# mhnazeri/PMoE

Hardware: AMD Instinct MI355X
Metric: samples/sec fwd+bwd, 256x256 RGB 4-expert PMoE (higher is better)
Workload: dtype bf16; 1 GPU; 4-expert MoE (PMoE experts), 256x256x3 x4 frames, batch 64/GPU, fwd+moe_loss+bwd, dropout 0.3; global_batch=64, parallelism=dp1

## Files before the change

pmoe_amd/csrc/api.hip:

```cpp
#include "common.h"
#include "kernels.h"

static ConvArgs to_args(const pmoe_conv_desc* d) {
    ConvArgs a;
    a.in = d->in; a.w = d->w; a.out = d->out; a.res = d->res; a.bias = d->bias; a.stats = d->stats;
    a.N = d->n; a.H = d->h; a.W = d->w_; a.Cin = d->cin;
    a.Ho = d->ho; a.Wo = d->wo; a.Cout = d->cout; a.CoutP = d->coutp;
    a.in_ld = d->in_ld; a.in_coff = d->in_coff; a.out_ld = d->out_ld; a.out_coff = d->out_coff;
    a.res_ld = d->res_ld; a.res_coff = d->res_coff;
    a.ipe = d->ipe; a.in_shared = d->in_shared;
    a.ks = d->ks; a.stride = d->stride; a.pad = d->pad; a.dilate = d->dilate;
    a.act = d->act; a.res_mode = (d->res || d->res_mode == PMOE_RES_INBN) ? d->res_mode : PMOE_RES_NONE;
    a.drop_p = d->drop_p; a.seed = d->seed;
    a.oscale = d->out_scale; a.in_scale = d->in_scale; a.w_fp8 = d->w_fp8; a.in_fp8 = d->in_fp8;
    a.bn = d->bn_coef; a.bn_ipe = d->bn_ipe > 0 ? d->bn_ipe : d->ipe;
    a.lTW = a.lTH = a.TN = a.n_groups = a.tiles_y = a.tiles_x = 0;
    a.kh = a.kw = d->ks; a.use_tapmap = 0; a.tapmap[0] = a.tapmap[1] = a.tapmap[2] = a.tapmap[3] = 0;
    a.out_step = 1; a.out_offy = a.out_offx = 0; a.OH = d->ho; a.OW = d->wo; a.prefetch = 0; a.stagger = 0;
    a.shuf_c = d->shuffle_c > 0 ? d->shuffle_c : 0;
    return a;
}

static int check_conv(const pmoe_conv_desc* d) {
    if (!d || !d->in || !d->w || !d->out) return PMOE_ERR_ARG;
    if (d->n <= 0 || d->h <= 0 || d->w_ <= 0 || d->ho <= 0 || d->wo <= 0 || d->ipe <= 0) return PMOE_ERR_ARG;
    const int ve = d->dtype == PMOE_DT_BF16 ? 8 : 4;
    if (d->in_fp8 && (!d->w_fp8 || d->dtype != PMOE_DT_BF16 || d->in_ld % 16 || d->in_coff % 16)) return PMOE_ERR_ARG;
    if (d->in_ld % ve || d->in_coff % ve || d->out_ld % ve || d->out_coff % ve) return PMOE_ERR_ARG;
    if (d->res && (d->res_ld % ve || d->res_coff % ve)) return PMOE_ERR_ARG;
    if (d->shuffle_c > 0 ? (d->cout != 4 * d->shuffle_c || d->shuffle_c % ve || d->out_coff + d->shuffle_c > d->out_ld || d->cout > d->coutp)
                         : (d->cout > d->coutp || d->out_coff + d->cout > d->out_ld)) return PMOE_ERR_ARG;
    if (d->in_coff + d->cin > d->in_ld) return PMOE_ERR_ARG;
    if (d->drop_p < 0.f || d->drop_p >= 1.f) return PMOE_ERR_ARG;
    if (d->res && d->res_mode == PMOE_RES_DBN &&
        (!d->bn_coef || !d->stats || d->dtype != PMOE_DT_BF16 || (d->bn_ipe > 0 && (d->bn_ipe % d->ipe || d->n % d->bn_ipe))))
        return PMOE_ERR_ARG;
    if (d->res_mode == PMOE_RES_INBN &&
        (d->res || !d->bn_coef || d->dtype != PMOE_DT_BF16 || (d->bias && d->ks != 1) || d->act != PMOE_ACT_NONE || d->drop_p != 0.f || d->in_shared ||
         d->w_fp8 || d->dilate || (d->bn_ipe > 0 && (d->bn_ipe % d->ipe || d->n % d->bn_ipe))))
        return PMOE_ERR_ARG;
    if (!d->dilate) {
        if (d->ho != (d->h + 2 * d->pad - d->ks) / d->stride + 1) return PMOE_ERR_ARG;
        if (d->wo != (d->w_ + 2 * d->pad - d->ks) / d->stride + 1) return PMOE_ERR_ARG;
    }
    return 0;
}

extern "C" {

int pmoe_version(void) { return PMOE_ABI_VERSION; }

int pmoe_abi_sizeof(int which) {
    return which == 0 ? (int)sizeof(pmoe_conv_desc) : which == 1 ? (int)sizeof(pmoe_wgrad_desc)
           : which == 2 ? (int)sizeof(pmoe_opt_tensor) : which == 3 ? (int)sizeof(pmoe_opt_pack)
           : which == 4 ? (int)sizeof(pmoe_aug_plan) : PMOE_ERR_ARG;
}

const char* pmoe_error_string(int code) {
    if (code == 0) return "ok";
    if (code == PMOE_ERR_ARG) return "pmoe: invalid argument (shape / alignment / pointer)";
    if (code == PMOE_ERR_UNSUPPORTED) return "pmoe: unsupported configuration (no tile fits LDS)";
    if (code > 0) return hipGetErrorString((hipError_t)code);
    return "pmoe: unknown error";
}

int pmoe_conv2d_igemm(const pmoe_conv_desc* d, void* stream) {
    int rc = check_conv(d);
    if (rc) return rc;
    return conv_igemm_launch(to_args(d), d->dtype, (hipStream_t)stream);
}

static ConvArgs to_plan_args(const pmoe_conv_desc* d) {
    ConvArgs a = to_args(d);
    if (a.in_ld <= 0) a.in_ld = a.in_coff + a.Cin;
    if (a.out_ld <= 0) a.out_ld = a.out_coff + a.Cout;
    return a;
}

int pmoe_conv2d_stat_rows(const pmoe_conv_desc* d) {
    if (!d || d->ipe <= 0) return PMOE_ERR_ARG;
    return conv_igemm_mblocks(to_plan_args(d), d->dtype);
}

int pmoe_conv2d_plan(const pmoe_conv_desc* d) {
    if (!d || d->ipe <= 0) return PMOE_ERR_ARG;
    return conv_igemm_plan(to_plan_args(d), d->dtype);
}

static int to_wgrad_args(const pmoe_wgrad_desc* d, WgradArgs& a) {
    if (!d || d->ipe <= 0) return PMOE_ERR_ARG;
    const int ve = d->dtype == PMOE_DT_BF16 ? 8 : 4;
    if (d->x_ld % ve || d->x_coff % ve || d->dy_ld % ve || d->dy_coff % ve) return PMOE_ERR_ARG;
    if (d->x_coff + d->cin > d->x_ld || d->dy_coff + d->cout > d->dy_ld) return PMOE_ERR_ARG;
// ... 47 lines not shown
```

pmoe_amd/csrc/conv_c16.hip:

```cpp
#include "common.h"
#include "kernels.h"

namespace {

typedef unsigned v4u __attribute__((ext_vector_type(4)));
typedef float f32x2 __attribute__((ext_vector_type(2)));

__global__ void __launch_bounds__(256, 2) conv3x3_c16_kernel(ConvArgs a, int tiles_x, int tiles_per_expert, int wgs_per_expert,
                                                            unsigned in_bytes, unsigned out_bytes) {
    __shared__ v4i wl[18][64];
    __shared__ v4i tbuf[4][256];
    __shared__ float red[4][8][2][64];
    const int tid = threadIdx.x, lane = tid & 63;
    const int wave = __builtin_amdgcn_readfirstlane(tid >> 6);
    const int e = blockIdx.y, wg = blockIdx.x;
    {
        const bf16* w = reinterpret_cast<const bf16*>(a.w) + (size_t)e * a.CoutP * 9 * 16;
        for (int idx = tid; idx < 18 * 64; idx += 256) {
            const int l = idx & 63, mtap = idx >> 6, mt = mtap / 9, tap = mtap - mt * 9;
            const int m = l & 31, kh = l >> 5;
            const int aa = m >> 3, hh = (m >> 2) & 1, b = m & 3;
            const int cout = 16 * (2 * mt + (aa >> 1)) + 8 * hh + 4 * (aa & 1) + b;
            wl[mtap][l] = ldg16(w + ((size_t)cout * 9 + tap) * 16 + kh * 8);
        }
    }
    __syncthreads();
    const size_t in_img0 = a.in_shared ? 0 : (size_t)e * a.ipe, out_img0 = (size_t)e * a.ipe;
    const __amdgpu_buffer_rsrc_t rs_in = __builtin_amdgcn_make_buffer_rsrc(
        (void*)(reinterpret_cast<const bf16*>(a.in) + in_img0 * a.H * a.W * a.in_ld + a.in_coff - a.in_ld), (short)0,
        (int)(in_bytes + (unsigned)a.in_ld * 2u), 0x00020000);
    const __amdgpu_buffer_rsrc_t rs_out = __builtin_amdgcn_make_buffer_rsrc(
        (void*)(reinterpret_cast<bf16*>(a.out) + out_img0 * a.H * a.W * a.out_ld + a.out_coff), (short)0, (int)out_bytes, 0x00020000);
    constexpr unsigned OOB = 0xfffffff0u;
    const int px_l = lane & 31, kh = lane >> 5;
    const unsigned ld2 = (unsigned)a.in_ld * 2u, old2 = (unsigned)a.out_ld * 2u;
    const unsigned vin = (unsigned)(px_l + 1) * ld2 + (unsigned)kh * 16u;
    unsigned vout[4];
#pragma unroll
    for (int i = 0; i < 4; ++i) vout[i] = (unsigned)(i * 8 + (lane >> 3)) * old2 + (unsigned)(lane & 7) * 16u;
    const bool chunk_ok = (lane & 7) * 8 < a.Cout;
    const int t0 = (int)((long long)tiles_per_expert * wg / wgs_per_expert);
    const int t1 = (int)((long long)tiles_per_expert * (wg + 1) / wgs_per_expert);
    f32x2 s1[4], s2[4];
#pragma unroll
    for (int j = 0; j < 4; ++j) s1[j] = s2[j] = f32x2{0.f, 0.f};

    struct Pos { int xt, y, img; };
    auto advance = [&](Pos& p) {
        p.xt += 4;
        while (p.xt >= tiles_x) { p.xt -= tiles_x; if (++p.y == a.H) { p.y = 0; ++p.img; } }
    };
    auto load_tile = [&](const Pos& p, v4u (&raw)[9], bool live) {
        const unsigned row0 = ((unsigned)(p.img * a.H + p.y) * (unsigned)a.W + (unsigned)p.xt * 32u) * ld2;
        const int px = p.xt * 32 + px_l;
        unsigned vq[3];
        vq[0] = live && px >= 1 && px - 1 < a.W ? vin - ld2 : OOB;
        vq[1] = live && px < a.W ? vin : OOB;
        vq[2] = live && px + 1 < a.W ? vin + ld2 : OOB;
#pragma unroll
        for (int r = 0; r < 3; ++r) {
            const int yy = p.y + r - 1;
            const bool row_ok = live && (unsigned)yy < (unsigned)a.H;
            const unsigned soff = row_ok ? row0 + (unsigned)(r - 1) * (unsigned)a.W * ld2 : 0u;
#pragma unroll
            for (int q = 0; q < 3; ++q)
                raw[r * 3 + q] = __builtin_amdgcn_raw_buffer_load_b128(rs_in, (int)(row_ok ? vq[q] : OOB), (int)soff, 0);
        }
    };
    auto process = [&](const Pos& pc, const v4u (&cur)[9]) {
        f32x16 acc[2];
#pragma unroll
        for (int mt = 0; mt < 2; ++mt)
#pragma unroll
            for (int i = 0; i < 16; ++i) acc[mt][i] = 0.f;
#pragma unroll
        for (int tap = 0; tap < 9; ++tap)
#pragma unroll
            for (int mt = 0; mt < 2; ++mt)
                acc[mt] = __builtin_amdgcn_mfma_f32_32x32x16_bf16(__builtin_bit_cast(bf16x8, wl[mt * 9 + tap][lane]),
                                                                  __builtin_bit_cast(bf16x8, cur[tap]), acc[mt], 0, 0, 0);
#pragma unroll
        for (int g = 0; g < 4; ++g) {
            float v[8];
#pragma unroll
            for (int i = 0; i < 8; ++i) v[i] = acc[g >> 1][8 * (g & 1) + i];
            tbuf[wave][px_l * 8 + ((2 * g + kh) ^ (px_l & 7))] = pack16<bf16>(v);
        }
        const unsigned osoff = ((unsigned)(pc.img * a.H + pc.y) * (unsigned)a.W + (unsigned)pc.xt * 32u) * old2;
#pragma unroll
        for (int i = 0; i < 4; ++i) {
            const int p = i * 8 + (lane >> 3), c = lane & 7;
            const v4i v = tbuf[wave][p * 8 + (c ^ (p & 7))];
            const bool ok = pc.xt * 32 + p < a.W;
            __builtin_amdgcn_raw_buffer_store_b128(__builtin_bit_cast(v4u, v), rs_out, (int)(ok && chunk_ok ? vout[i] : OOB), (int)osoff, 0);
            if (a.stats && ok) {
                float rr[8];
                unpack16<bf16>(v, rr);
#pragma unroll
                for (int q = 0; q < 4; ++q) {
                    const f32x2 r2 = f32x2{rr[2 * q], rr[2 * q + 1]};
                    s1[q] += r2;
                    s2[q] = __builtin_elementwise_fma(r2, r2, s2[q]);
                }
            }
        }
    };
    Pos pl, pc;
    {
        const int t = t0 + wave;
        pl.xt = t % tiles_x;
        const int r = t / tiles_x;
        pl.y = r % a.H;
        pl.img = r / a.H;
        pc = pl;
    }
    v4u b0[9], b1[9], b2[9];
    int tl = t0 + wave, t = tl;
    auto fetch = [&](v4u (&buf)[9]) {
        load_tile(pl, buf, tl < t1);
        advance(pl);
        tl += 4;
    };
    fetch(b0);
    fetch(b1);
    while (t < t1) {
        fetch(b2);
        process(pc, b0); advance(pc); t += 4;
        if (t >= t1) break;
        fetch(b0);
        process(pc, b1); advance(pc); t += 4;
        if (t >= t1) break;
        fetch(b1);
        process(pc, b2); advance(pc); t += 4;
    }
    if (!a.stats) return;
#pragma unroll
    for (int q = 0; q < 8; ++q) {
        red[wave][lane >> 3][0][(lane & 7) * 8 + q] = s1[q >> 1][q & 1];
        red[wave][lane >> 3][1][(lane & 7) * 8 + q] = s2[q >> 1][q & 1];
    }
    __syncthreads();
    if (tid < 128) {
        const int which = tid >> 6, c = tid & 63;
        float s = 0.f;
        for (int w = 0; w < 4; ++w)
            for (int pg = 0; pg < 8; ++pg) s += red[w][pg][which][c];
        a.stats[(((size_t)e * wgs_per_expert + wg) * 2 + which) * a.CoutP + c] = s;
    }
}

}

bool conv_c16_plan(const ConvArgs& a, int dtype, ConvLaunch* l) {
    if (!sw("PMOE_CONV_C16", 1)) return false;
    if (dtype != PMOE_DT_BF16 || a.w_fp8 || a.ks != 3 || a.stride != 1 || a.pad != 1 || a.dilate) return false;
    if (a.Cin != 16 || a.CoutP != 64 || a.Cout % 8 || a.Cout > 64) return false;
    if (a.bias || a.act != PMOE_ACT_NONE || a.res_mode != PMOE_RES_NONE || a.drop_p > 0.f) return false;
    if (a.N % a.ipe || a.Ho != a.H || a.Wo != a.W) return false;
    if (a.in_ld % 8 || a.in_coff % 8 || a.out_ld % 8 || a.out_coff % 8) return false;
    if ((long long)a.ipe * a.H * a.W * (a.in_ld > a.out_ld ? a.in_ld : a.out_ld) * 2 >= 0xfff00000ll) return false;
    const int E = a.N / a.ipe, tx = (a.W + 31) / 32;
    const long long tpe = (long long)a.ipe * a.H * tx;
    if (tpe > 0x7fffffffll || tpe < 64) return false;
    int wpe = 512 / E;
    if (wpe < 1) wpe = 1;
    if (wpe > tpe / 16) wpe = (int)(tpe / 16);
    if (wpe < 1) wpe = 1;
    l->kind = CONV_C16; l->code = 1316; l->a = a;
    l->wpe = wpe; l->tiles_x = tx; l->tpe = (int)tpe; l->mblocks = E * wpe;
    return true;
}

int conv_c16_launch(const ConvLaunch& l, hipStream_t st) {
    const ConvArgs& a = l.a;
    const long long in_b = (long long)a.ipe * a.H * a.W * a.in_ld * 2 - (long long)a.in_coff * 2;
    const long long out_b = (long long)a.ipe * a.H * a.W * a.out_ld * 2 - (long long)a.out_coff * 2;
    return launch<conv3x3_c16_kernel, 0>(dim3(l.wpe, a.N / a.ipe), dim3(256), 0, st, a, l.tiles_x, l.tpe, l.wpe, (unsigned)in_b, (unsigned)out_b);
}
```

pmoe_amd/csrc/conv_igemm.hip:

```cpp
#include "conv_common.h"
#include <stdlib.h>
#include <string.h>
#include "kernels.h"

template <int LOG_RB> __device__ __forceinline__ int swz(int x) { return swz_chunk<LOG_RB, 0>(x); }

template <typename T> struct Mma;
template <> struct Mma<bf16> {
    static __device__ __forceinline__ void run(const v4i& a, const v4i& b, f32x16& c) {
        c = __builtin_amdgcn_mfma_f32_32x32x16_bf16(__builtin_bit_cast(bf16x8, a), __builtin_bit_cast(bf16x8, b), c, 0, 0, 0);
    }
};
template <> struct Mma<float> {
    static __device__ __forceinline__ void run(const v4i& a, const v4i& b, f32x16& c) {
        const f32x4 fa = __builtin_bit_cast(f32x4, a), fb = __builtin_bit_cast(f32x4, b);
#pragma unroll
        for (int j = 0; j < 4; ++j) c = __builtin_amdgcn_mfma_f32_32x32x2f32(fa[j], fb[j], c, 0, 0, 0);
    }
};

template <> struct Mma<fp8> {
    static __device__ __forceinline__ void run(const v4i& a, const v4i& b, f32x16& c) {
        typedef long l2 __attribute__((ext_vector_type(2)));
        const l2 la = __builtin_bit_cast(l2, a), lb = __builtin_bit_cast(l2, b);
// ... 404 lines not shown
        l->smem = smem;
        l->log_rb = log_rb; l->lite = lite;
        l->wm = big || !wide ? 4 : 2; l->wn = wide ? 2 : 1;
        l->code = (F8 ? 8000 : 0) + (lite ? 2000 + log_rb : log_rb * 100 + l->wm * 10 + l->wn);
        return 0;
    }
    return PMOE_ERR_UNSUPPORTED;
}

static int tile_plan_dtype(const ConvArgs& a, int dtype, ConvLaunch* l) {
    return dtype == PMOE_DT_BF16 ? tile_plan(a, 2, 2, l) : dtype == PMOE_DT_F32 ? tile_plan(a, 4, 4, l) : PMOE_ERR_ARG;
}

template <typename T, typename TL = T> static int tile_launch(const ConvLaunch& l, hipStream_t st) {
    const ConvArgs& a = l.a;
    if (l.lite) return launch_lite<T, 7, TL>(a, l.mblocks, l.smem, st);
    switch (l.log_rb * 100 + l.wm * 10 + l.wn) {
    case 742: return launch_cfg<T, 7, 4, 2, TL>(a, l.mblocks, l.smem, st);
    case 642: return launch_cfg<T, 6, 4, 2, TL>(a, l.mblocks, l.smem, st);
    case 722: return launch_cfg<T, 7, 2, 2, TL>(a, l.mblocks, l.smem, st);
    case 741: return launch_cfg<T, 7, 4, 1, TL>(a, l.mblocks, l.smem, st);
    case 622: return launch_cfg<T, 6, 2, 2, TL>(a, l.mblocks, l.smem, st);
    case 641: return launch_cfg<T, 6, 4, 1, TL>(a, l.mblocks, l.smem, st);
    }
    if constexpr (sizeof(TL) == sizeof(T)) {
        switch (l.log_rb * 100 + l.wm * 10 + l.wn) {
        case 542: return launch_cfg<T, 5, 4, 2>(a, l.mblocks, l.smem, st);
        case 522: return launch_cfg<T, 5, 2, 2>(a, l.mblocks, l.smem, st);
        case 541: return launch_cfg<T, 5, 4, 1>(a, l.mblocks, l.smem, st);
        }
    }
    return PMOE_ERR_UNSUPPORTED;
}

static int launch_one(const ConvLaunch& l, int dtype, hipStream_t st) {
    switch (l.kind) {
    case CONV_SKINNY: return gemm_skinny_launch(l, st);
    case CONV_C16: return conv_c16_launch(l, st);
    case CONV_C1X1: return conv_c1x1_launch(l, st);
    case CONV_RES: return conv_res_launch(l, st);
    case CONV_DMA: case CONV_DMA_S2: case CONV_DMA_S2CLS: case CONV_DMA_F8: return conv_dma_launch(l, st);
    case CONV_TILE:
        if (l.a.w_fp8) return !l.a.oscale || !(l.a.in_scale > 0.f) ? PMOE_ERR_ARG : tile_launch<bf16, fp8>(l, st);
        return dtype == PMOE_DT_BF16 ? tile_launch<bf16>(l, st) : tile_launch<float>(l, st);
    }
    return PMOE_ERR_ARG;
}

static int select_stride2_dgrad(const ConvArgs& a, int dtype, ConvPlan* p) {
    p->n = 0;
    for (int py = 0; py < 2; ++py)
        for (int px = 0; px < 2; ++px) {
            ConvArgs c = a;
            c.dilate = 0; c.stride = 1; c.pad = 0;
            c.kh = 1 + py; c.kw = 1 + px;
            c.Ho = (a.Ho - py + 1) / 2; c.Wo = (a.Wo - px + 1) / 2;
            if (c.Ho <= 0 || c.Wo <= 0) continue;
            c.OH = a.Ho; c.OW = a.Wo; c.out_step = 2; c.out_offy = py; c.out_offx = px;
            c.use_tapmap = 1;
            for (int r = 0; r < c.kh; ++r)
                for (int q = 0; q < c.kw; ++q) {
                    const int fy = py ? (r == 0 ? 0 : 2) : 1, fx = px ? (q == 0 ? 0 : 2) : 1;
                    c.tapmap[r * c.kw + q] = fy * 3 + fx;
                }
            ConvLaunch* l = &p->l[p->n++];
            if (!conv_dma_s2cls_plan(c, dtype, l)) {
                const int rc = tile_plan_dtype(c, dtype, l);
                if (rc) return rc;
            }
        }
    if (!p->n) return PMOE_ERR_ARG;
    ConvLaunch t;
    const int esz = dtype == PMOE_DT_BF16 ? 2 : 4, rc = tile_plan(a, esz, esz, &t);
    p->mblocks = rc ? rc : t.mblocks;
    return 4000 + p->l[p->n - 1].code;
}

int conv_select(const ConvArgs& a, int dtype, ConvPlan* p) {
    memset(p, 0, sizeof(*p));
    p->n = 1;
    ConvLaunch* l = p->l;
    int code = 0;
    const bool bn_mode = a.res_mode == PMOE_RES_INBN || a.res_mode == PMOE_RES_DBN;
    if (a.in_fp8 && !a.w_fp8) {
        code = PMOE_ERR_UNSUPPORTED;
    } else if (a.shuf_c) {
        code = conv_c1x1_plan(a, dtype, l) ? 0 : PMOE_ERR_UNSUPPORTED;
    } else if (a.w_fp8) {
        if (dtype != PMOE_DT_BF16 || a.dilate) code = PMOE_ERR_ARG;
        else if (a.in_fp8) code = conv_dma_f8_plan(a, dtype, l) ? 0 : PMOE_ERR_UNSUPPORTED;
        else if (bn_mode) code = PMOE_ERR_UNSUPPORTED;
        else code = tile_plan(a, 2, 1, l);
    } else if (a.res_mode == PMOE_RES_INBN) {
        if (!(!a.bias && conv_res_plan(a, dtype, l) && l->res_pipe) && !conv_c1x1_plan(a, dtype, l))
            code = PMOE_ERR_UNSUPPORTED;
    } else if (a.res_mode == PMOE_RES_DBN) {
        if (!(conv_res_plan(a, dtype, l) && l->res_dma) && (gemm_skinny_plan(a, dtype, l) || !conv_dma_plan(a, dtype, l)))
            code = PMOE_ERR_UNSUPPORTED;
    } else if (a.dilate && a.ks == 3 && a.pad == 1 && a.kh == 3) {
        const int code = select_stride2_dgrad(a, dtype, p);
        if (code < 0) p->n = 0;
        return p->code = code;
    } else if (a.dilate && a.ks == 1 && a.pad == 0 && a.res_mode == PMOE_RES_ADD && a.res == a.out && a.res_ld == a.out_ld &&
               a.res_coff == a.out_coff && !a.bias && a.act == PMOE_ACT_NONE && a.drop_p == 0.f) {
        ConvArgs c = a;
        c.dilate = 0; c.stride = 1; c.pad = 0; c.kh = c.kw = 1;
        c.Ho = (a.Ho + 1) / 2; c.Wo = (a.Wo + 1) / 2;
        c.OH = a.Ho; c.OW = a.Wo; c.out_step = 2; c.out_offy = c.out_offx = 0;
        code = tile_plan_dtype(c, dtype, l);
    } else if (!gemm_skinny_plan(a, dtype, l) && !conv_c16_plan(a, dtype, l) && !conv_c1x1_plan(a, dtype, l) &&
               !conv_res_plan(a, dtype, l) && !conv_dma_plan(a, dtype, l) && !conv_dma_s2_plan(a, dtype, l)) {
        code = tile_plan_dtype(a, dtype, l);
    }
    if (code < 0) { p->n = 0; return p->code = code; }
    p->mblocks = l->mblocks;
    return p->code = l->code;
}

int conv_igemm_launch(const ConvArgs& a, int dtype, hipStream_t st) {
    ConvPlan p;
    const int code = conv_select(a, dtype, &p);
    if (code < 0) return code;
    for (int i = 0; i < p.n; ++i) {
        const int rc = launch_one(p.l[i], dtype, st);
        if (rc) return rc;
    }
    return 0;
}

int conv_igemm_plan(const ConvArgs& a, int dtype) {
    ConvPlan p;
    return conv_select(a, dtype, &p);
}

int conv_igemm_mblocks(const ConvArgs& a, int dtype) {
    static float rows_only;
    ConvArgs s = a;
    if (!s.stats) s.stats = &rows_only;
    ConvPlan p;
    const int code = conv_select(s, dtype, &p);
    return code < 0 ? code : p.mblocks;
}
```

pmoe_amd/engine.py:

```python
import collections
import itertools
import os

import torch
import torch.distributed as dist

from . import hip, ops
from .model import blocks as B
from .parallel import BucketedAllReduce

F32 = torch.float32


def r16(c):
    return (c + 15) // 16 * 16


def r64(c):
    return (c + 63) // 64 * 64


class BNCoef:
    __slots__ = ("block", "mean", "invstd", "scale", "shift", "rpe")

    def __init__(self, E, C_, rpe, dev):
        self.block, self.rpe = torch.empty(4, E, C_, dtype=F32, device=dev), rpe
        self.mean, self.invstd, self.scale, self.shift = self.block.unbind(0)


class Partials(collections.namedtuple("Partials", "t rows E")):
    __slots__ = ()

    @classmethod
    def of_epilogue(cls, stats, E):
        return cls(stats, stats.shape[0] // E, E)

    def fold(self, width, cap=128):
        if self.rows <= cap:
            return self
        small = torch.empty(self.E, 128, width, dtype=F32, device=self.t.device)
        ops.reduce_partials(self.t, small, self.E, self.rows, 128, width)
        return Partials(small, 128, self.E)


BNSource = collections.namedtuple("BNSource", "z layer coef")
BNFused = collections.namedtuple("BNFused", "g coef c1 c2")


class Var:
    __slots__ = ("t", "coff", "c", "g", "needs_grad", "act", "drop_p", "base", "gap_part", "bn_src", "bn_part", "f8", "bn_defer",
                 "bn_fused", "pending_bn", "sink")

    def __init__(self, t, c=None, coff=0, needs_grad=False, base=None):
        self.t, self.coff, self.c = t, coff, (c if c is not None else t.shape[-1])
        self.g, self.needs_grad, self.act, self.drop_p, self.base = None, needs_grad, hip.ACT_NONE, 0.0, base
        self.gap_part = None
        self.bn_src = None
        self.bn_part = None
        self.f8 = None
        self.bn_defer = False
        self.bn_fused = None
        self.pending_bn = None
        self.sink = None

    @property
    def grad(self):
        return self.base.g if self.base is not None else self.g

    def set_grad(self, g):
        if (self.base if self.base is not None else self).bn_part is not None:
            raise RuntimeError("relu(BatchNorm(z)) whose backward reductions came out of its consumer's data gradient "
                               "(PMOE_RES_DBN) takes exactly one consumer; a second gradient contribution arrived")
        if self.base is not None:
            self.base.g = g
        else:
            self.g = g

    def window(self, coff, c):
        return Var(self.t, c, coff, self.needs_grad, base=self if self.base is None else self.base)


PackSinks = collections.namedtuple("PackSinks", "gen by_param")


class GroupedConv:
    scatter_grads = None
    route_bias = True

    def __init__(self, eng, name, weights, biases, cin, cout, ks, stride, pad):
        self.eng, self.name = eng, name
        self.weights, self.biases = weights, biases
        self.cin, self.cout, self.ks, self.stride, self.pad = cin, cout, ks, stride, pad
        self.cinp, self.coutp, self.cout_st = r16(cin), r64(cout), r16(cout)
        self.dg_rows, self.dg_red = r64(cin), r16(cout)
# ... 874 lines not shown
        self._arena_numel = (off + 255) // 256 * 256

    def _bucket_cuts(self, n_buckets):
        tail = None
        for key in self._order:
            layer = next((l for k, l, _ in self.params if self._key(k, l) == key), None)
            name = getattr(layer, "name", "")
            if name.startswith("layer1.") or name.startswith("stem.") or name in ("bn1", "eca1", "eca2"):
                tail = self._slots[key][0]
                break
        n = self._arena_numel
        if tail is None or tail <= 0 or n_buckets < 2:
            b = (n + n_buckets - 1) // n_buckets
            return [min(n, (i + 1) * ((b + 255) // 256 * 256)) for i in range(n_buckets)]
        tail = tail // 256 * 256
        b = (tail + n_buckets - 2) // (n_buckets - 1)
        b = (b + 255) // 256 * 256
        return [min(tail, (i + 1) * b) for i in range(n_buckets - 1)] + [n]

    def _grad_slot(self, kind, layer):
        key = self._key(kind, layer)
        off, n, _ = self._slots[key]
        self._filled.add(key)
        return self._arena[off:off + n]

    def _final_prefix(self):
        while self._cursor < len(self._order):
            key = self._order[self._cursor]
            _, _, plist = self._slots[key]
            if key in self._filled or not any(p.requires_grad for p in plist):
                self._cursor += 1
            else:
                break
        if self._cursor == len(self._order):
            return self._arena_numel
        return self._slots[self._order[self._cursor]][0]

    def _begin(self, images, training, taping, dtype, base_seed):
        if images.dim() != 5:
            raise ValueError(f"images: expected [B,T,C,H,W], got {tuple(images.shape)}")
        if not images.is_cuda:
            raise RuntimeError("pmoe_amd: inputs must be on the MI355X (cuda) device; there is no CPU path")
        hip.load()
        self.dev, self.dtype = images.device, dtype
        self.training, self.taping = training, taping
        self.base_seed = int(base_seed)
        Bsz = images.shape[0]
        self.B, self.N = Bsz, Bsz * self.E
        self._ensure_built(self.dev, dtype)
        self._refresh_tables(self.dev)
        self._pack_all()
        self.tape, self._bn_touched = [], []
        self._seed_counter = itertools.count(1)
        return Bsz

    def prepare(self, images, dtype):
        Bsz = self._begin(images, False, False, dtype, 0)
        self.tape = None
        return Bsz

    def forward(self, images, speed, command, training, taping, dtype, base_seed=0, in_grads=None):
        self._in_grads = tuple(bool(w) for w in in_grads) if in_grads is not None else (False, False, False)
        if any(self._in_grads) and not taping:
            raise RuntimeError("input gradients need the backward tape")
        Bsz = self._begin(images, training, taping, dtype, base_seed)
        x0 = self._image_input(images)
        spd, cmd = self._measurement_inputs(speed, command)

        feat = Var(self._new(self.N, 1, 1, 1536))
        self._backbone_fwd(x0, feat)
        self._mlp(spd, self.speed_enc, out=feat, out_coff=512, in_shared=True)
        self._mlp(cmd, self.cmd_enc, out=feat, out_coff=1024, in_shared=True)
        return self._heads_fwd(feat, Bsz, training)

    def _backbone_fwd(self, x0, feat):
        H, W = x0.t.shape[1], x0.t.shape[2]
        hw_ok = H * W >= 256
        fold2 = self.fold_eca_gate and hw_ok and self.conv2.cin % 64 == 0
        want_dx = self._in_grads[0]
        if want_dx and not hw_ok:
            raise NotImplementedError("the gradient with respect to images needs frames of at least 256 pixels (its gate term comes "
                                      "from the per-image filter gradients)")
        if self.taping and hw_ok and (want_dx or (self.fold_stem_input and (self.conv1.trainable or self.eca1.trainable))):
            x0s, gate, gapmean = self._eca(x0, self.eca1, shared=True, tape=False)
            z1, st = self._conv_stats(x0s, self.conv1, tape=False)
            z1.needs_grad = True
            z1.bn_defer = (self.training and self.dtype == torch.bfloat16 and not want_dx
                           and fold2 and ops.conv2d_wgrad_bn_served(z1.t.shape[0], H, W, z1.t.shape[1], z1.t.shape[2], self.conv1.cinp,
                                                                    self.conv1.cout_st, 64, 64, self.B, 3, 1, self.conv1.pad, self.dtype,
                                                                    x_ld=x0.t.shape[-1], dy_ld=z1.t.shape[-1], x_shared=True,
                                                                    per_image=True))
            self.tape.append(lambda: self._stem_in_bwd(x0, z1, gate, gapmean))
            a1 = self._bn(z1, self.bn_c1, relu=True, stats=st, want_gap=fold2)
        else:
            x0s = self._eca(x0, self.eca1, shared=True)
            a1 = self._conv_bn(x0s, self.conv1, self.bn_c1, relu=True)
        if fold2:
            z2, st = self._eca_conv_folded(a1, self.eca2, self.conv2)
        else:
            a1s = self._eca(a1, self.eca2, shared=False)
            z2, st = self._conv_stats(a1s, self.conv2)
        if self.fuse_stem_tail:
            o = self._stem_tail(z2, st)
        else:
            a2 = self._bn(z2, self.bn_c2, relu=True, stats=st)
            a3 = self._bn(a2, self.bn1, relu=True)
            o = self._maxpool(a3)
        for bi, blk in enumerate(self.blocks):
            idn = o
            if blk["down"] is not None:
                idn = self._conv_bn(o, blk["down"][0], blk["down"][1], relu=False)
            nxt = self.blocks[bi + 1]["conv1"] if bi + 1 < len(self.blocks) else None
            aA = self._conv_bn(o, blk["conv1"], blk["bn1"], relu=True, want_f8=blk["conv2"].fp8)
            o = self._conv_bn(aA, blk["conv2"], blk["bn2"], relu=True, res=idn, want_f8=nxt is not None and nxt.fp8)
        self._gap_to(o, feat, 0)

    def _conv_bn(self, x, conv, bn, relu, res=None, out=None, want_f8=False, pool_to=None):
        if self.training or self.taping or not self.fold_bn_eval or conv.w_f8 is not None:
            z, st = self._conv_stats(x, conv)
            return self._bn(z, bn, relu=relu, res=res, stats=st, out=out, want_f8=want_f8, pool_to=pool_to)
        E = self.E
        key = (self.dtype, str(self.dev)) + tuple(p._version for p in conv.weights) + tuple(
            v for m in bn.mods for v in (m.weight._version, m.bias._version, m.running_mean._version, m.running_var._version))
        cache = conv.__dict__.get("_bn_fold")
        if cache is None or cache[0] != key:
            k = self._bn_coeffs(bn, 1)
            wf = torch.empty(E, conv.coutp, conv.taps, conv.cinp, dtype=self.dtype, device=self.dev)
            bf = torch.empty(E, conv.coutp, dtype=F32, device=self.dev)
            ops.pack_conv_weights_scaled(self._tab("w", conv), k.scale, k.shift, k.mean, wf, bf, E, conv.cout, conv.cin, conv.ks,
                                         conv.coutp, conv.cinp, self.dtype)
            cache = conv.__dict__["_bn_fold"] = (key, wf, bf)
        _, wf, bf = cache
        Ho, Wo, o = self._conv_out(x, conv, out)
        ops.set_meta(flop=2.0 * self.N * Ho * Wo * conv.cout * conv.cin * conv.taps, name=conv.name + "+bn")
        ops.conv2d(x.t, wf, o.t, cin=conv.cinp, cout=conv.cout_st, coutp=conv.coutp, ipe=self.B, ks=conv.ks,
                   stride=conv.stride, pad=conv.pad, in_shared=(x.t.shape[0] != self.N), in_coff=x.coff, out_coff=o.coff,
                   bias=bf,
                   act=hip.ACT_RELU if relu else hip.ACT_NONE, res=res.t if res is not None else None,
                   res_coff=res.coff if res is not None else 0, res_mode=hip.RES_ADD)
        return o

    def _heads_fwd(self, feat, Bsz, training):
        E = self.E
        sp = self._mlp(feat, self.speed_pred)
        af = self._mlp(feat, self.action_feat)
        if self.alt:
            head = self._conv(af, self.head)
            al = self._mlp(feat, self.alpha_mlp)
            head5 = self._merge_alt_head(head, al)
        else:
            head5 = self._conv(af, self.head)
        K = self.K
        probs = torch.empty(Bsz, K, dtype=F32, device=self.dev)
        mean = torch.empty(Bsz, K, 2, dtype=F32, device=self.dev)
        std = torch.empty(Bsz, K, 2, dtype=F32, device=self.dev)
        speeds = torch.empty((Bsz, 1) if self.shared else (Bsz, K, 1), dtype=F32, device=self.dev)
        ops.gate_mixture_fwd(head5.t.view(self.N, -1), sp.t.view(self.N, 16), probs, mean, std, speeds, Bsz, K,
                             self._alpha_mode(), self.shared)
        self._bump_batch_counters()
        state = dict(tape=self.tape, tail=(head5, sp, probs), B=self.B, N=self.N, dev=self.dev, dtype=self.dtype,
                     in_names=[n for n, want in zip(("images", "speed", "command"), self._in_grads) if want])
        self.tape = None
        return probs, mean, std, speeds, state

    def _alpha_mode(self):
        return int(not self.alt and not self.shared) | (2 if self.raw_alpha else 0)

    def _measurement_inputs(self, speed, command):
        Bsz = self.B
        if speed.shape != (Bsz, self.speed_enc["layers"][0].cin) or command.shape != (Bsz, self.cmd_enc["layers"][0].cin):
            raise ValueError("speed / command shapes do not match the encoders")
        spd = Var(self._new(Bsz, 1, 1, 16))
        ops.pad_rows(speed.contiguous().float(), spd.t.view(Bsz, 16))
        cmd = Var(self._new(Bsz, 1, 1, 16))
        ops.pad_rows(command.contiguous().float(), cmd.t.view(Bsz, 16))
        for v, name, want in ((spd, "speed", self._in_grads[1]), (cmd, "command", self._in_grads[2])):
            if want:
                v.sink, v.needs_grad = name, True
        return spd, cmd

    def _bump_batch_counters(self):
        if not self._bn_touched:
            return
        count, layers = {}, {}
        for l in self._bn_touched:
            count[id(l)] = count.get(id(l), 0) + 1
            layers[id(l)] = l
        tensors = [m.num_batches_tracked for k, l in layers.items() for m in l.mods]
        steps = [count[k] for k, l in layers.items() for _ in l.mods]
        torch._foreach_add_(tensors, steps)
        torch.autograd.graph.increment_version([b for l in layers.values() for m in l.mods
                                                for b in (m.running_mean, m.running_var)])

    def _image_input(self, images):
        Bsz, (H, W) = images.shape[0], images.shape[-2:]
        cin = images.shape[1] * images.shape[2]
        if cin != self.conv1.cin:
            raise ValueError(f"images carry {cin} channels (T*C), the backbone stem expects {self.conv1.cin}")
        x0 = Var(self._new(Bsz, H, W, r16(cin)))
        ops.nchw_to_nhwc(images.reshape(Bsz, cin, H, W).contiguous().float(), x0.t)
        return x0

    @property
    def _epilogue_stats(self):
        return self.training and self.fuse_conv_stats and self.dtype == torch.bfloat16

    def _conv_stats(self, x, layer, tape=True, in_bn=None):
        if self._epilogue_stats:
            return self._conv(x, layer, bias=False, want_stats=True, tape=tape, in_bn=in_bn)
        return self._conv(x, layer, bias=False, tape=tape, in_bn=in_bn), None

    def _stem_in_bwd(self, x0, z1, gate, gapmean):
        dy = z1.grad
        if dy is None:
            return
        layer = self.conv1
        ops.set_meta(flop=2.0 * self.N * dy.shape[1] * dy.shape[2] * layer.cout * layer.cin * layer.taps, name=layer.name,
                     bytes=(2 if z1.bn_fused is not None else 1) * dy.numel() * dy.element_size())
        f = z1.bn_fused
        fuse = (z1.t, f.coef.block, f.c1, f.c2) if f is not None else None
        want_dx = self._in_grads[0]
        H, W = dy.shape[1], dy.shape[2]
        if not want_dx:
            self._filter_grads(x0.t, dy, layer, self.eca1, gate, gapmean, x_shared=True, bn_fuse=fuse)
            return
        dgap = self._filter_grads(x0.t, dy, layer, self.eca1, gate, gapmean, want_dgap=True, dgap_scale=1.0 / (H * W),
                                  x_shared=True, bn_fuse=fuse)
        wd = torch.empty(self.N, layer.dg_rows, layer.taps, layer.dg_red, dtype=self.dtype, device=self.dev)
        ops.pack_conv_weights_gated(self._tab("w", layer), gate, None, wd, self.N, self.B, layer.cout, layer.cin, layer.ks,
                                    layer.coutp, layer.cinp, layer.dg_rows, layer.dg_red, self.dtype)
        dx = torch.empty(self.B, layer.cin, H, W, dtype=F32, device=self.dev)
        ops.set_meta(flop=2.0 * self.N * H * W * layer.cout * layer.cinp * layer.taps, name=layer.name + ":dinput",
                     bytes=dy.numel() * dy.element_size() + dx.numel() * 4)
        ops.stem_input_grad(dy, wd, dgap, dx, self.E)
        self._input_grads["images"] = dx
        if self.debug_input_grad is not None:
            self.debug_input_grad.update(dz1=dy, wd=wd, dgap=dgap, dx=dx)

    def _filter_grads(self, xt, dy, layer, ecal, gate, gapmean, want_dgap=False, dgap_scale=1.0, **wgrad_kw):
        N, B_, E, c = self.N, self.B, self.E, gate.shape[-1]
        cow, cpw = self._wgrad_tile(layer)
        G = self._wgrad_ws(N * layer.taps * cow * cpw, main=True)
        ops.conv2d_wgrad(xt, dy, G, cin=layer.cinp, cout=layer.cout_st, cinp=cpw, coutp=cow, ipe=B_, ks=layer.ks,
                         stride=layer.stride, pad=layer.pad, per_image=True, **wgrad_kw)
        ds = torch.empty(N, c, dtype=F32, device=self.dev)
        dw = self._grad_slot("w", layer) if layer.trainable else torch.empty(
            E * layer.cout * layer.cin * layer.taps, dtype=F32, device=self.dev)
        ops.eca_stem_fold(G, gate, self._tab("w", layer), dw, ds, N, B_, layer.cout, layer.cin, layer.ks, cow, cpw)
        dgap = torch.empty(N, c, dtype=F32, device=self.dev) if want_dgap else None
        if ecal.trainable or want_dgap:
            dwe = self._grad_slot("eca", ecal).view(E, ecal.k) if ecal.trainable else torch.empty(
                E, ecal.k, dtype=F32, device=self.dev)
            ops.eca_bwd_small(ds, 1, gate, gapmean, self._tab("eca", ecal), ecal.k, dgap, dwe, N, B_, c, ecal.creal,
                              dgap_scale=dgap_scale)
        return dgap

    def _merge_alt_head(self, head, al):
        merged = Var(torch.empty_like(head.t))
        ops.copy_window(head.t, 0, merged.t, 0, 16)
        ops.copy_window(al.t, 0, merged.t, 4, 1)
        merged.needs_grad = head.needs_grad or al.needs_grad
        if self.taping and merged.needs_grad:
            def bwd():
                g = merged.grad
                if g is None:
                    return
                gh = g.clone()
                gh.view(self.N, 16)[:, 4] = 0
                head.set_grad(gh)
                ga = torch.zeros_like(al.t)
                ga.view(self.N, 16)[:, 0] = g.view(self.N, 16)[:, 4]
                al.set_grad(ga)
            self.tape.append(bwd)
        return merged

    def _tail_bwd(self, tail, dprobs, dmean, dstd, dspeeds):
        head5, sp, probs = tail
        dhead = torch.empty_like(head5.t)
        dspd = torch.empty_like(sp.t)

        def c(t):
            return t.contiguous().float() if t is not None else None
        ops.gate_mixture_bwd(head5.t.view(self.N, -1), probs, c(dprobs), c(dmean), c(dstd), c(dspeeds),
                             dhead.view(self.N, -1), dspd.view(self.N, 16), self.B, self.K,
                             self._alpha_mode(), self.shared)
        if dprobs is not None or dmean is not None or dstd is not None:
            head5.set_grad(dhead)
        if dspeeds is not None:
            sp.set_grad(dspd)

    def backward(self, tape_state, *douts):
        tape = tape_state["tape"]
        self.B, self.N, self.dev, self.dtype = (tape_state[k] for k in ("B", "N", "dev", "dtype"))
# ... 38 lines not shown
```

pmoe_amd/ops.py:

```python
import ctypes as C

import torch

from . import hip
from .hip import ConvDesc, WgradDesc, check, dt, load, ptr, stream_ptr


def _round_up(v, m):
    return (v + m - 1) // m * m


def conv_out_size(h, ks, stride, pad):
    return (h + 2 * pad - ks) // stride + 1


def _nhwc(t, name):
    if t.dim() != 4:
        raise ValueError(f"{name}: expected NHWC [N,H,W,C], got shape {tuple(t.shape)}")
    return t.shape


def _conv_desc(n, h, w_, ho, wo, cin, cout, coutp, ipe, ks, stride, pad, dtype, *, dilate=False, in_shared=False, in_ld=0,
               in_coff=0, out_ld=0, out_coff=0, res_mode=hip.RES_NONE, res_ld=0, res_coff=0, act=hip.ACT_NONE, drop_p=0.0, seed=0,
               w_fp8=False, in_fp8=False, in_scale=1.0, bn_ipe=0, shuffle2_c=0):
# ... 30 lines not shown
    d.bias, d.stats = (7 if bias else None), (8 if stats else None)
    return d


class ConvLaunch:
    __slots__ = ("d", "out", "stats")

    def __init__(self, d, out, stats):
        self.d, self.out, self.stats = d, out, stats

    def plan(self):
        return load().pmoe_conv2d_plan(C.byref(self.d))

    def served(self):
        return self.plan() >= 0

    def stat_rows(self):
        return _stat_rows(self.d)

    def launch(self):
        return _conv2d_launch(self)


def _stat_rows(d):
    rows = load().pmoe_conv2d_stat_rows(C.byref(d))
    if rows < 0:
        check(rows, "pmoe_conv2d_stat_rows")
    return rows


def _conv2d_launch(p):
    d = p.d
    if p.out is None:
        raise ValueError("conv2d: a launch prepared from shapes only can be asked, not run")
    if p.stats is not None:
        rows = p.stat_rows()
        if p.stats is True:
            p.stats = torch.empty(rows, 2, d.coutp, dtype=torch.float32, device=p.out.device)
        elif p.stats.dim() != 3 or p.stats.shape[0] != rows or p.stats.shape[1] != 2 or p.stats.shape[2] != d.coutp:
            raise ValueError(f"conv2d: stats must be [{rows}, 2, {d.coutp}] for this launch, got {tuple(p.stats.shape)}")
        d.stats = ptr(p.stats, "stats", torch.float32)
    elif d.res_mode == hip.RES_DBN:
        raise ValueError("conv2d: RES_DBN writes the BatchNorm-backward reductions to `stats`")
    if _prof is not None:
        _launch_info["kernel"] = p.plan()
    check(load().pmoe_conv2d_igemm(C.byref(d), stream_ptr()), "pmoe_conv2d_igemm")
    return p.out


def conv2d_prepare(x, w_packed, out, *, cin, cout, coutp, ipe, ks, stride, pad, dilate=False, in_shared=False,
                   in_coff=0, out_coff=0, res=None, res_coff=0, res_mode=hip.RES_NONE, bias=None, act=hip.ACT_NONE,
                   drop_p=0.0, seed=0, stats=None, out_scale=None, in_scale=1.0, bn_coef=None, bn_ipe=0, shuffle2_c=0,
                   shapes_only=False):
    at = _stand_in if shapes_only else ptr
    nin, h, w_, ldx = _nhwc(x, "x")
    n, ho, wo, ldo = _nhwc(out, "out")
    if shuffle2_c:
        if ho % 2 or wo % 2 or ks != 1 or cout != 4 * shuffle2_c:
            raise ValueError("conv2d: shuffle2_c needs a 1x1 layer with 4 * shuffle2_c outputs and an even-sided destination")
        ho, wo = ho // 2, wo // 2
    w_fp8 = w_packed.dtype == torch.uint8
    in_fp8 = w_fp8 and x.dtype == torch.uint8
    if (x.dtype != out.dtype and not in_fp8) or (w_packed.dtype != out.dtype and not w_fp8):
        raise ValueError("conv2d: x, w and out must share one dtype")
    if w_fp8 and (out_scale is None or out.dtype != torch.bfloat16):
        raise ValueError("conv2d: e4m3 weights need bf16 activations and the per-channel out_scale of the pack")
    in_, w, o = at(x, "x"), at(w_packed, "w"), at(out, "out")
    res_p, bias_p = at(res, "res", out.dtype), at(bias, "bias", torch.float32)
    stats_p = C.c_void_p(8) if stats is True else at(stats, "stats", torch.float32)
    d = _conv_desc(n, h, w_, ho, wo, cin, cout, coutp, ipe, ks, stride, pad, dt(out), dilate=dilate, in_shared=in_shared,
                   in_ld=ldx, in_coff=in_coff, out_ld=ldo, out_coff=out_coff,
                   res_mode=res_mode if (res is not None or res_mode == hip.RES_INBN) else hip.RES_NONE,
                   res_ld=res.shape[-1] if res is not None else 0, res_coff=res_coff, act=act, drop_p=drop_p, seed=seed,
                   w_fp8=w_fp8, in_fp8=in_fp8, in_scale=in_scale, bn_ipe=bn_ipe, shuffle2_c=shuffle2_c)
    d.in_, d.w, d.out, d.res, d.bias, d.stats = in_, w, o, res_p, bias_p, stats_p
    if w_fp8:
        d.out_scale = at(out_scale, "out_scale", torch.float32)
    if d.res_mode in (hip.RES_DBN, hip.RES_INBN):
        inbn = d.res_mode == hip.RES_INBN
        want = (4, n // (bn_ipe or ipe), cin if inbn else cout)
        if (inbn and res is not None) or bn_coef is None or bn_coef.dtype != torch.float32 or tuple(bn_coef.shape) != want:
            raise ValueError(f"conv2d: RES_{'INBN takes no `res` and' if inbn else 'DBN'} needs bn_coef {list(want)} f32")
        d.bn_coef = at(bn_coef, "bn_coef", torch.float32)
    if in_shared and nin != ipe:
        raise ValueError("conv2d: shared input must hold exactly ipe images")
    if not in_shared and nin != n:
        raise ValueError("conv2d: input/output image counts differ")
    if w_packed.numel() < (n // ipe) * coutp * ks * ks * cin:
        raise ValueError("conv2d: packed weight tensor too small")
    return ConvLaunch(d, None if shapes_only else out, stats)


def conv2d(x, w_packed, out, *, plan_only=False, **kw):
    if kw.get("stats") is True:
        raise ValueError("conv2d: stats=True (the launch allocates the buffer) is conv2d_prepare's: conv2d returns only `out`")
    p = conv2d_prepare(x, w_packed, out, **kw)
    return p.plan() if plan_only else p.launch()


def conv2d_plan(n, h, w_, ho, wo, cin, cout, coutp, ipe, ks, stride, pad, dtype, *, bias=False, stats=False, **kw):
    return load().pmoe_conv2d_plan(C.byref(_planning_desc(n, h, w_, ho, wo, cin, cout, coutp, ipe, ks, stride, pad, dtype,
                                                          bias=bias, stats=stats, **kw)))


def conv2d_stat_rows(n, h, w_, ho, wo, cin, cout, coutp, ipe, ks, stride, pad, dtype, w_fp8=False, in_ld=0, out_ld=0,
                     in_shared=False, in_fp8=False):
    return _stat_rows(_planning_desc(n, h, w_, ho, wo, cin, cout, coutp, ipe, ks, stride, pad, dtype, w_fp8=w_fp8, in_fp8=in_fp8,
                                     in_ld=in_ld, out_ld=out_ld, in_shared=in_shared))


_wgrad_scratch = {}


def _wgrad_part_ws(device, floats):
    key = (device, torch.cuda.current_stream(device).cuda_stream)
    buf = _wgrad_scratch.get(key)
    if buf is None or buf.numel() < floats:
        buf = _wgrad_scratch[key] = torch.empty(max(floats, 1 << 22), dtype=torch.float32, device=device)
    return buf


def _wgrad_desc(n, h, w_, ho, wo, cin, cout, cinp, coutp, ipe, ks, stride, pad, dtype, *, x_ld=0, dy_ld=0, x_coff=0, dy_coff=0,
                x_shared=False, per_image=False, bn_z_ld=None):
    d = WgradDesc()
    d.n, d.h, d.w_, d.cin, d.cinp = n, h, w_, cin, cinp
    d.ho, d.wo, d.cout, d.coutp = ho, wo, cout, coutp
    d.x_ld, d.x_coff, d.dy_ld, d.dy_coff = x_ld or x_coff + cin, x_coff, dy_ld or dy_coff + cout, dy_coff
    d.ipe, d.x_shared = ipe, int(x_shared)
    d.ks, d.stride, d.pad, d.dtype = ks, stride, pad, dtype
    d.per_image = int(per_image)
    if bn_z_ld is not None:
        d.bn_fused, d.bn_z_ld = 1, bn_z_ld or d.dy_ld
    return d


def _wgrad_ws(d):
    need = load().pmoe_conv2d_wgrad_ws_floats(C.byref(d))
    if need < 0:
        check(int(need), "pmoe_conv2d_wgrad_ws_floats")
    return need, max(1, need // ((d.n // d.ipe) * d.ks * d.ks * d.coutp * d.cinp))


def conv2d_wgrad_bn_served(n, h, w_, ho, wo, cin, cout, cinp, coutp, ipe, ks, stride, pad, dtype, *, bn_z_ld=0, **kw):
    d = _wgrad_desc(n, h, w_, ho, wo, cin, cout, cinp, coutp, ipe, ks, stride, pad, hip._TORCH_DT[dtype], bn_z_ld=bn_z_ld, **kw)
    return load().pmoe_conv2d_wgrad_plan(C.byref(d)) >= 0


def conv2d_wgrad_nsplit(n, h, w_, ho, wo, cin, cout, cinp, coutp, ipe, ks, stride, pad, dtype, **kw):
    return _wgrad_ws(_wgrad_desc(n, h, w_, ho, wo, cin, cout, cinp, coutp, ipe, ks, stride, pad, hip._TORCH_DT[dtype], **kw))[1]


def conv2d_wgrad(x, dy, dw_ws, *, cin, cout, cinp, coutp, ipe, ks, stride, pad, x_shared=False, x_coff=0, dy_coff=0,
                 per_image=False, plan_only=False, grads=None, grads_cout=0, grads_cin=0, defer_fold=False, bn_fuse=None):
    nin, h, w_, ldx = _nhwc(x, "x")
    n, ho, wo, ldy = _nhwc(dy, "dy")
    d = _wgrad_desc(n, h, w_, ho, wo, cin, cout, cinp, coutp, ipe, ks, stride, pad, dt(x), x_ld=ldx, dy_ld=ldy, x_coff=x_coff,
                    dy_coff=dy_coff, x_shared=x_shared, per_image=per_image, bn_z_ld=None if bn_fuse is None else bn_fuse[0].shape[-1])
    d.x, d.dy = ptr(x, "x"), ptr(dy, "dy", x.dtype)
    d.dw_ws = ptr(dw_ws, "dw_ws", torch.float32) if dw_ws is not None else None
    if bn_fuse is not None:
        z, coef, c1, c2 = bn_fuse
        if z.shape[:3] != dy.shape[:3]:
            raise ValueError("conv2d_wgrad: bn_fuse z must have the geometry of dy")
        if not plan_only:
            E_ = n // ipe
            if coef.shape != (4, E_, cout) or c1.shape != (E_, cout) or c2.shape != (E_, cout):
                raise ValueError("conv2d_wgrad: bn_fuse coefficient blocks must be [4,E,cout] / [E,cout]")
            d.bn_z, d.bn_coef = ptr(z, "bn_z", x.dtype), ptr(coef, "bn_coef", torch.float32)
            d.bn_c1, d.bn_c2 = ptr(c1, "bn_c1", torch.float32), ptr(c2, "bn_c2", torch.float32)
    if grads is not None:
        if per_image or grads.dtype != torch.float32 or grads.numel() != (n // ipe) * grads_cout * grads_cin * ks * ks:
            raise ValueError("conv2d_wgrad: grads must hold E * cout * cin * ks * ks float32 values (not with per_image)")
        d.grads, d.cout_real, d.cin_real = ptr(grads, "grads", torch.float32), int(grads_cout), int(grads_cin)
    if bn_fuse is not None and plan_only:
        return load().pmoe_conv2d_wgrad_plan(C.byref(d))
    if dw_ws.numel() < (n if per_image else n // ipe) * ks * ks * coutp * cinp:
        raise ValueError("conv2d_wgrad: workspace too small")
    need, nsplit = _wgrad_ws(d)
    if plan_only:
        return nsplit
    if need > 0:
        part = _wgrad_part_ws(x.device, need)
        d.part_ws, d.part_ws_floats = ptr(part, "part_ws"), part.numel()
    if _prof is not None:
        _launch_info["kernel"] = load().pmoe_conv2d_wgrad_plan(C.byref(d))
    d.defer_fold = int(defer_fold)
    check(load().pmoe_conv2d_wgrad(C.byref(d), stream_ptr()), "pmoe_conv2d_wgrad")
    return d if defer_fold else dw_ws


def mlp_wgrad(x, dy, grads, bias_grads, *, cin, cout, cin_real, cout_real, ipe, x_shared=False, x_coff=0, dy_coff=0):
# ... 616 lines not shown
```

Baseline: 1911 samples/s.

## Fold stem ECA gate into per-image weights over a shared frame bank

```diff
diff --git a/pmoe_amd/csrc/api.hip b/pmoe_amd/csrc/api.hip
--- a/pmoe_amd/csrc/api.hip
+++ b/pmoe_amd/csrc/api.hip
@@ -8,7 +8,7 @@
     a.Ho = d->ho; a.Wo = d->wo; a.Cout = d->cout; a.CoutP = d->coutp;
     a.in_ld = d->in_ld; a.in_coff = d->in_coff; a.out_ld = d->out_ld; a.out_coff = d->out_coff;
     a.res_ld = d->res_ld; a.res_coff = d->res_coff;
-    a.ipe = d->ipe; a.in_shared = d->in_shared;
+    a.ipe = d->ipe; a.in_shared = d->in_shared == d->ipe ? 1 : d->in_shared;
     a.ks = d->ks; a.stride = d->stride; a.pad = d->pad; a.dilate = d->dilate;
     a.act = d->act; a.res_mode = (d->res || d->res_mode == PMOE_RES_INBN) ? d->res_mode : PMOE_RES_NONE;
     a.drop_p = d->drop_p; a.seed = d->seed;
diff --git a/pmoe_amd/csrc/conv_c16.hip b/pmoe_amd/csrc/conv_c16.hip
--- a/pmoe_amd/csrc/conv_c16.hip
+++ b/pmoe_amd/csrc/conv_c16.hip
@@ -25,7 +25,7 @@
         }
     }
     __syncthreads();
-    const size_t in_img0 = a.in_shared ? 0 : (size_t)e * a.ipe, out_img0 = (size_t)e * a.ipe;
+    const size_t in_img0 = a.in_shared > 1 ? (size_t)(e % a.in_shared) : a.in_shared ? 0 : (size_t)e * a.ipe, out_img0 = (size_t)e * a.ipe;
     const __amdgpu_buffer_rsrc_t rs_in = __builtin_amdgcn_make_buffer_rsrc(
         (void*)(reinterpret_cast<const bf16*>(a.in) + in_img0 * a.H * a.W * a.in_ld + a.in_coff - a.in_ld), (short)0,
         (int)(in_bytes + (unsigned)a.in_ld * 2u), 0x00020000);
@@ -161,7 +161,9 @@
     if ((long long)a.ipe * a.H * a.W * (a.in_ld > a.out_ld ? a.in_ld : a.out_ld) * 2 >= 0xfff00000ll) return false;
     const int E = a.N / a.ipe, tx = (a.W + 31) / 32;
     const long long tpe = (long long)a.ipe * a.H * tx;
-    if (tpe > 0x7fffffffll || tpe < 64) return false;
+    const bool banks = a.in_shared > 1;
+    if (banks && a.ipe != 1) return false;
+    if (tpe > 0x7fffffffll || (tpe < 64 && !banks)) return false;
     int wpe = 512 / E;
     if (wpe < 1) wpe = 1;
     if (wpe > tpe / 16) wpe = (int)(tpe / 16);
diff --git a/pmoe_amd/csrc/conv_igemm.hip b/pmoe_amd/csrc/conv_igemm.hip
--- a/pmoe_amd/csrc/conv_igemm.hip
+++ b/pmoe_amd/csrc/conv_igemm.hip
@@ -510,7 +510,11 @@
     ConvLaunch* l = p->l;
     int code = 0;
     const bool bn_mode = a.res_mode == PMOE_RES_INBN || a.res_mode == PMOE_RES_DBN;
-    if (a.in_fp8 && !a.w_fp8) {
+    if (a.in_shared < 0 || (a.in_shared > 1 && (a.in_shared % a.ipe || a.N % a.in_shared))) {
+        code = PMOE_ERR_ARG;
+    } else if (a.in_shared > 1) {
+        if (a.in_fp8 || a.shuf_c || bn_mode || !conv_c16_plan(a, dtype, l)) code = PMOE_ERR_UNSUPPORTED;
+    } else if (a.in_fp8 && !a.w_fp8) {
         code = PMOE_ERR_UNSUPPORTED;
     } else if (a.shuf_c) {
         code = conv_c1x1_plan(a, dtype, l) ? 0 : PMOE_ERR_UNSUPPORTED;
diff --git a/pmoe_amd/engine.py b/pmoe_amd/engine.py
--- a/pmoe_amd/engine.py
+++ b/pmoe_amd/engine.py
@@ -10,6 +10,7 @@
 from .parallel import BucketedAllReduce
 
 F32 = torch.float32
+STEM_FOLD_MIN_BYTES = 256 << 20
 
 
 def r16(c):
@@ -1050,8 +1051,12 @@
             raise NotImplementedError("the gradient with respect to images needs frames of at least 256 pixels (its gate term comes "
                                       "from the per-image filter gradients)")
         if self.taping and hw_ok and (want_dx or (self.fold_stem_input and (self.conv1.trainable or self.eca1.trainable))):
-            x0s, gate, gapmean = self._eca(x0, self.eca1, shared=True, tape=False)
-            z1, st = self._conv_stats(x0s, self.conv1, tape=False)
+            folded = self._stem_in_folded(x0) if self._stem_fold_pays(x0) else None
+            if folded is not None:
+                z1, st, gate, gapmean = folded
+            else:
+                x0s, gate, gapmean = self._eca(x0, self.eca1, shared=True, tape=False)
+                z1, st = self._conv_stats(x0s, self.conv1, tape=False)
             z1.needs_grad = True
             z1.bn_defer = (self.training and self.dtype == torch.bfloat16 and not want_dx
                            and fold2 and ops.conv2d_wgrad_bn_served(z1.t.shape[0], H, W, z1.t.shape[1], z1.t.shape[2], self.conv1.cinp,
@@ -1061,8 +1066,14 @@
             self.tape.append(lambda: self._stem_in_bwd(x0, z1, gate, gapmean))
             a1 = self._bn(z1, self.bn_c1, relu=True, stats=st, want_gap=fold2)
         else:
-            x0s = self._eca(x0, self.eca1, shared=True)
-            a1 = self._conv_bn(x0s, self.conv1, self.bn_c1, relu=True)
+            bn_passes = self.training or self.taping or not self.fold_bn_eval or self.conv1.w_f8 is not None
+            untaped = not (self.taping and (self.conv1.trainable or self.eca1.trainable))
+            folded = self._stem_in_folded(x0) if hw_ok and bn_passes and untaped and self._stem_fold_pays(x0) else None
+            if folded is not None:
+                a1 = self._bn(folded[0], self.bn_c1, relu=True, stats=folded[1])
+            else:
+                x0s = self._eca(x0, self.eca1, shared=True)
+                a1 = self._conv_bn(x0s, self.conv1, self.bn_c1, relu=True)
         if fold2:
             z2, st = self._eca_conv_folded(a1, self.eca2, self.conv2)
         else:
@@ -1177,6 +1188,37 @@
         if self._epilogue_stats:
             return self._conv(x, layer, bias=False, want_stats=True, tape=tape, in_bn=in_bn)
         return self._conv(x, layer, bias=False, tape=tape, in_bn=in_bn), None
+
+    def _stem_fold_pays(self, x0):
+        B_, h, w, c = x0.t.shape
+        return self.E * B_ * h * w * c * x0.t.element_size() > STEM_FOLD_MIN_BYTES
+
+    def _stem_in_folded(self, x0):
+        layer, ecal = self.conv1, self.eca1
+        B_, h, w, c = x0.t.shape
+        N = self.N
+        if self.dtype != torch.bfloat16 or h * w < 256 or layer.w_f8 is not None or B_ != self.B:
+            return None
+        if layer.cinp != 16:
+            return None
+        Ho, Wo = (ops.conv_out_size(s, layer.ks, layer.stride, layer.pad) for s in (h, w))
+        kw = dict(cin=layer.cinp, cout=layer.cout_st, coutp=layer.coutp, ipe=1, ks=layer.ks, stride=layer.stride, pad=layer.pad,
+                  in_shared=B_, stats=True if self._epilogue_stats else None)
+        if not ops.conv2d_banks_served(N, B_, h, w, Ho, Wo, layer.cinp, layer.cout_st, layer.coutp, layer.ks, layer.stride, layer.pad,
+                                       self.dtype, stats=self._epilogue_stats, in_ld=c, out_ld=layer.cout_st):
+            return None
+        gap = self._gap_sums(x0)
+        gate = torch.empty(N, c, dtype=F32, device=self.dev)
+        gapmean = torch.empty(N, c, dtype=F32, device=self.dev)
+        ops.eca_gate(gap.t, gap.rows, h * w, self._tab("eca", ecal), ecal.k, gate, gapmean, N, B_, B_, c, ecal.creal)
+        wf = torch.empty(N, layer.coutp, layer.taps, layer.cinp, dtype=self.dtype, device=self.dev)
+        ops.pack_conv_weights_gated(self._tab("w", layer), gate, wf, None, N, B_, layer.cout, layer.cin, layer.ks, layer.coutp,
+                                    layer.cinp, layer.dg_rows, layer.dg_red, self.dtype)
+        o = self._conv_out(x0, layer)[2]
+        run = ops.conv2d_prepare(x0.t, wf, o.t, **kw)
+        ops.set_meta(flop=2.0 * N * Ho * Wo * layer.cout * layer.cin * layer.taps, name=layer.name)
+        run.launch()
+        return o, (Partials.of_epilogue(run.stats, self.E) if run.stats is not None else None), gate, gapmean
 
     def _stem_in_bwd(self, x0, z1, gate, gapmean):
         dy = z1.grad
diff --git a/pmoe_amd/ops.py b/pmoe_amd/ops.py
--- a/pmoe_amd/ops.py
+++ b/pmoe_amd/ops.py
@@ -136,8 +136,8 @@
         if (inbn and res is not None) or bn_coef is None or bn_coef.dtype != torch.float32 or tuple(bn_coef.shape) != want:
             raise ValueError(f"conv2d: RES_{'INBN takes no `res` and' if inbn else 'DBN'} needs bn_coef {list(want)} f32")
         d.bn_coef = at(bn_coef, "bn_coef", torch.float32)
-    if in_shared and nin != ipe:
-        raise ValueError("conv2d: shared input must hold exactly ipe images")
+    if in_shared and nin != (ipe if int(in_shared) == 1 else int(in_shared)):
+        raise ValueError("conv2d: shared input must hold exactly ipe (in_shared = S > 1: S) images")
     if not in_shared and nin != n:
         raise ValueError("conv2d: input/output image counts differ")
     if w_packed.numel() < (n // ipe) * coutp * ks * ks * cin:
@@ -161,6 +161,11 @@
                      in_shared=False, in_fp8=False):
     return _stat_rows(_planning_desc(n, h, w_, ho, wo, cin, cout, coutp, ipe, ks, stride, pad, dtype, w_fp8=w_fp8, in_fp8=in_fp8,
                                      in_ld=in_ld, out_ld=out_ld, in_shared=in_shared))
+
+
+def conv2d_banks_served(n, frames, h, w_, ho, wo, cin, cout, coutp, ks, stride, pad, dtype, *, stats=False, in_ld=0, out_ld=0):
+    return load().pmoe_conv2d_plan(C.byref(_planning_desc(n, h, w_, ho, wo, cin, cout, coutp, 1, ks, stride, pad, dtype, stats=stats,
+                                                          in_shared=frames, in_ld=in_ld, out_ld=out_ld))) >= 0
 
 
 _wgrad_scratch = {}
```

After: 1911 samples/s (median of 2 runs). Within noise of the previous version (-0.0%).
